# lh3/bfc

Measured on AMD Instinct MI355X. Metric: M k-mers/s counted (bloom+htab) on 150 bp reads, higher is better.
Workload: dtype u64

## Files before the change

bfc_amd/csrc/bfcg_bloom3.hip:

```cpp
#include <hip/hip_runtime.h>
#include <stdint.h>
#include <stdlib.h>
#include "kmer_dev.h"
#include "bfcg_internal.h"
#include "bfcg_dev.h"

using namespace bfcg;

#define B3_UND 0x40000000u
#define B3_SEEN16 0x8000u
#define B3_COLD_NR 8
#define B3_WALK_U 4
template <int BT, int PF, bool COLD>
__global__ __launch_bounds__(BT, PF <= 2 ? 8 : 6) void k_bloom3(KParams P, BloomArgs A)
{
	extern __shared__ __attribute__((aligned(16))) unsigned char smem[];
	__shared__ uint32_t s_list_n, s_ovf, s_pool_off, s_emit_n, s_fs_used, s_wb_n, s_pad3[2];
	const uint32_t f = blockIdx.x;
	const bool ho_log = A.ho_stride != 0;
#ifdef BFCG_MEASURE
	const long long t_start = clock64();
#endif
	const bool eager = A.eager != 0, spec = eager && A.cap2 != 0;
	constexpr int B3_SL = 1024 / BT;
	uint4 sl[B3_SL];
	uint32_t e_st = 0, e_f0 = 0, e_f2 = 0, e_c = 0, e_s = 0, e_h = 0;
	RecW<3> cur[PF], nxt[PF];
#pragma unroll
	for (int u = 0; u < PF; ++u) { cur[u].d[0] = cur[u].d[1] = cur[u].d[2] = 0; nxt[u] = cur[u]; }
#pragma unroll
	for (int j = 0; j < B3_SL; ++j) sl[j] = make_uint4(0, 0, 0, 0);
	if (eager) {
		const uint4 *src = reinterpret_cast<const uint4 *>(reinterpret_cast<const unsigned int *>(A.bloom) + (uint64_t)f * (16u << P.R));
#pragma unroll
		for (int j = 0; j < B3_SL; ++j) if ((uint32_t)(threadIdx.x + j * BT) < (4u << P.R)) sl[j] = src[threadIdx.x + j * BT];
		const uint32_t *const any = reinterpret_cast<const uint32_t *>(A.stats);
		const uint32_t *const p_st = A.sticky ? A.sticky : any, *const p_fl = A.flags ? A.flags : any;
		const uint32_t *const p_c = A.cnt2 ? A.cnt2 + f : A.start + f + 1, *const p_s = A.cap2 ? any : A.start + f, *const p_h = ho_log ? A.ho_cur + f : any;
		e_st = *p_st; e_f0 = p_fl[0]; e_f2 = p_fl[2]; e_c = *p_c; e_s = *p_s; e_h = *p_h;
		if (spec) {
			const uint32_t *r0 = A.recs + (uint64_t)(f * A.cap2) * 3;
#pragma unroll
			for (int u = 0; u < PF; ++u) { const uint32_t i = threadIdx.x + u * BT; if (i < A.cap2) cur[u] = rec_load<3>(r0 + (uint64_t)i * 3); }
		}
	}
	const bool poisoned = eager ? (((A.sticky ? e_st : 0u) | (A.flags ? e_f0 | e_f2 : 0u)) != 0u) : batch_poisoned(A);
	if (poisoned) { if (ho_log && threadIdx.x == 0) A.ho_mark[f] = A.ho_cur[f]; return; }
	uint32_t rs, n;
	if (!eager) region_list(A, f, rs, n);
	else if (A.cap2) { rs = f * A.cap2; n = e_c < A.cap2 ? e_c : A.cap2; }
	else { rs = e_s; n = A.cnt2 ? e_c : e_c - e_s; }
	if (n == 0) { if (threadIdx.x == 0) { if (ho_log) A.ho_mark[f] = A.ho_cur[f]; else if (A.agg_cnt) A.agg_cnt[f] = 0; } return; }
	uint32_t ho_cur0 = 0;
	unsigned long long *ho_base;
	if (ho_log) {
		ho_cur0 = eager ? e_h : A.ho_cur[f];
		if (ho_cur0 + n > A.ho_stride) {
			if (threadIdx.x == 0) { atomicAdd(&A.stats[(size_t)(f & (ST_SLOTS - 1)) * ST_N + ST_ERR_POOL], 1ULL); A.ho_mark[f] = ho_cur0; }
			return;
		}
		ho_base = A.ho + (uint64_t)f * A.ho_stride + ho_cur0;
	} else ho_base = reinterpret_cast<unsigned long long *>(A.stream_out) + rs;
	A.stats += (size_t)(f & (ST_SLOTS - 1)) * ST_N;
	const uint32_t region_dw = 16u << P.R;
	unsigned char *sp = smem;
	unsigned int *region = reinterpret_cast<unsigned int *>(sp); sp += (size_t)region_dw * 4;
	const uint32_t nblk = 1u << P.R;
	unsigned int *bcnt = reinterpret_cast<unsigned int *>(sp), *boff = bcnt + nblk;
	if (COLD) sp += (size_t)(2 * nblk + 4) * 4;
	unsigned int *fs = reinterpret_cast<unsigned int *>(sp); if (!COLD) sp += (size_t)P.fs_cap * 4;
	unsigned int *la = reinterpret_cast<unsigned int *>(sp); sp += (size_t)P.list_cap * 4;
	unsigned int *lb = reinterpret_cast<unsigned int *>(sp); sp += (size_t)P.list_cap * 4;
	unsigned short *lc = reinterpret_cast<unsigned short *>(sp); sp += (size_t)P.list_cap * 2;
	unsigned short *ord = reinterpret_cast<unsigned short *>(sp);
	const uint32_t fs_mask = P.fs_cap - 1;
	const uint32_t *recs = A.recs + (uint64_t)rs * 3;
	unsigned int *g_region = reinterpret_cast<unsigned int *>(A.bloom) + (uint64_t)f * region_dw;
	const uint32_t imp = (P.f_base + f) >> P.F2;
	const Dec3 D = dec3_geom(P);
	const int tid = threadIdx.x, lane = tid & 63;
	const uint32_t mask_a = (1u << D.a) - 1u, imp_sh = D.n ? imp << D.lo : 0u, sh_up = D.lo + D.n;
#ifdef BFCG_MEASURE
	const bool timing = BFCG_ABL(P, 64) && tid == 0;
	long long tq[7] = {0, 0, 0, 0, 0, 0, 0};
	long long tc[7] = {0, 0, 0, 0, 0, 0, 0};
	if (timing) tq[0] = t_start;
#define B3_TC(i) do { if (timing) tc[i] = clock64(); } while (0)
#else
#define B3_TC(i) do { } while (0)
#endif
	auto addr3 = [&](uint32_t d0, uint32_t d1) -> uint32_t {
		const uint32_t y0d = d0 & mask_a, upper = y0d >> D.up;
		const uint32_t y0lo = D.n ? (y0d & D.lowmask) | imp_sh | (upper << sh_up) : y0d;
		const uint32_t y1lo = __builtin_amdgcn_alignbit(d1, d0, D.a) & D.mk32;
		const uint32_t hh = upper | (((y0lo - y1lo) ^ y1lo) << D.sh_x);
		uint32_t h2 = (hh >> 9) & 511u;
		h2 |= (uint32_t)((h2 & 31u) == 0);
		return (y0d & D.rmask) | ((hh & 511u) << 8) | (h2 << 17);
	};
	auto entry3 = [&](uint32_t d0, uint32_t d1) -> unsigned long long {
		const unsigned long long AA = d0 | ((unsigned long long)d1 << 32);
		const unsigned long long y1 = (AA >> D.a) & ((1ULL << P.k) - 1);
		const uint32_t y0d = d0 & mask_a;
		const unsigned long long id = (unsigned long long)((y0d & D.rmask) | ((y0d >> D.up) << D.R)) | (y1 << D.sh_y1);
		return (id << 1) | (unsigned long long)((d1 >> D.sh_flag) & 1u);
	};
#pragma unroll
	for (int u = 0; u < PF; ++u) {
		const uint32_t i = tid + u * BT;
		if (!spec && i < n) cur[u] = rec_load<3>(recs + (uint64_t)i * 3);
		if (i + BT * PF < n) nxt[u] = rec_load<3>(recs + (uint64_t)(i + BT * PF) * 3);
	}
	if (spec) {
#pragma unroll
		for (int u = 0; u < PF; ++u) if ((uint32_t)(tid + u * BT) >= n) cur[u].d[0] = cur[u].d[1] = cur[u].d[2] = 0;
	}
	{
		const uint4 *src = reinterpret_cast<const uint4 *>(g_region);
		uint4 *dst = reinterpret_cast<uint4 *>(region);
		if (eager) {
#pragma unroll
			for (int j = 0; j < B3_SL; ++j) if ((uint32_t)(tid + j * BT) < region_dw / 4) dst[tid + j * BT] = sl[j];
		} else for (uint32_t i = tid; i < region_dw / 4; i += BT) dst[i] = src[i];
		if constexpr (COLD) { for (uint32_t i = tid; i < 2 * nblk + 4; i += BT) bcnt[i] = 0; }
		else {
			uint4 *f4 = reinterpret_cast<uint4 *>(fs);
			for (uint32_t i = tid; i < P.fs_cap / 4; i += BT) f4[i] = make_uint4(FS32_EMPTY, FS32_EMPTY, FS32_EMPTY, FS32_EMPTY);
		}
		if (tid == 0) { s_list_n = 0; s_emit_n = 0; s_ovf = 0; s_fs_used = 0; s_wb_n = 0; }
	}
	__syncthreads();
#ifdef BFCG_MEASURE
	if (timing) tq[1] = clock64();
#endif
	volatile uint32_t *v_ovf = &s_ovf;

	for (uint32_t base = 0; base < n; base += BT * PF) {
		uint32_t pk[PF], um[PF];
#pragma unroll
		for (int u = 0; u < PF; ++u) {
			pk[u] = 0; um[u] = 0;
			if (base + u * BT + (uint32_t)(tid & ~63) < n) {
				pk[u] = addr3(cur[u].d[0], cur[u].d[1]);
				const B3Pos b = b3_positions((pk[u] >> 8) & 511u, pk[u] >> 17);
				const uint32_t bl64 = (pk[u] & 255u) << 6;
				const uint32_t w0 = *b3_wordp(region, bl64, b.b0), w1 = *b3_wordp(region, bl64, b.b1), w2 = *b3_wordp(region, bl64, b.b2), w3 = *b3_wordp(region, bl64, b.b3);
				um[u] = (b3_bit(w0, b.b0) | (b3_bit(w1, b.b1) << 1) | (b3_bit(w2, b.b2) << 2) | (b3_bit(w3, b.b3) << 3)) ^ 15u;
			}
		}
		unsigned long long ms[PF], ml[PF];
// ... 22 lines not shown
					if constexpr (COLD) __hip_atomic_fetch_add(&bcnt[pk[u] & 255u], 1u, __ATOMIC_RELAXED, __HIP_MEMORY_SCOPE_WORKGROUP);
				}
			}
			o_s += (uint32_t)__popcll(ms[u]); o_l += (uint32_t)__popcll(ml[u]);
		}
		if (base + BT * PF < n) {
#pragma unroll
			for (int u = 0; u < PF; ++u) {
				cur[u] = nxt[u];
				const uint32_t i = base + 2 * BT * PF + tid + u * BT;
				if (i < n) nxt[u] = rec_load<3>(recs + (uint64_t)i * 3);
			}
		}
	}
	__syncthreads();
#ifdef BFCG_MEASURE
	if (timing) tq[2] = clock64();
#endif
	const uint32_t ln = s_list_n;
	const bool ovf_list = ln > P.list_cap || ln > (COLD ? (uint32_t)(B3_COLD_NR * BT) : 8191u) || n > 65535u;
	bool dirty = true;
	if constexpr (COLD) {
		if (!ovf_list) {
			B3_TC(0);
			if (tid < 64) {
				const uint32_t per = (nblk + 63u) >> 6, b0 = (uint32_t)tid * per;
				uint32_t v[4] = {0, 0, 0, 0}, sum = 0;
#pragma unroll
				for (int t = 0; t < 4; ++t) if ((uint32_t)t < per && b0 + t < nblk) { v[t] = bcnt[b0 + t]; sum += v[t]; }
				uint32_t inc = sum;
#pragma unroll
				for (int o = 1; o < 64; o <<= 1) { const uint32_t x = __shfl_up(inc, o); if (lane >= o) inc += x; }
				uint32_t run = inc - sum;
#pragma unroll
				for (int t = 0; t < 4; ++t) if ((uint32_t)t < per && b0 + t < nblk) { boff[b0 + t] = run; bcnt[b0 + t] = run; run += v[t]; }
				if (tid == 63) boff[nblk] = inc;
			}
// ... 31 lines not shown
					sx[t] = x; sw[t] = ((w >> 8) & 0x3ffffu) | (r << 18); sq[t] = lc[pos];
				}
			}
			__syncthreads();
			B3_TC(3);
#pragma unroll
			for (int t = 0; t < B3_COLD_NR; ++t) {
				if ((uint32_t)tid + (uint32_t)t * BT < ln) {
					const uint32_t r = sw[t] >> 18;
					const B3Pos b = b3_positions(sw[t] & 511u, (sw[t] >> 9) & 511u);
					la[r] = sx[t]; lb[r] = b.b0 | (b.b1 << 9) | (b.b2 << 18); ord[r] = (unsigned short)b.b3; lc[r] = (unsigned short)sq[t];
				}
			}
			__syncthreads();
			B3_TC(4);
			if ((uint32_t)tid < nblk) {
				const uint32_t bl = (uint32_t)tid, bl64 = bl << 6, s0 = boff[bl], s1 = boff[bl + 1], last = s1 - 1u;
				uint32_t pw_n[B3_WALK_U] = {0, 0, 0, 0}, p3_n[B3_WALK_U] = {0, 0, 0, 0};
				if (s0 < s1) {
#pragma unroll
					for (int u = 0; u < B3_WALK_U; ++u) { const uint32_t jj = min(s0 + (uint32_t)u, last); pw_n[u] = lb[jj]; p3_n[u] = ord[jj]; }
				}
				for (uint32_t j = s0; j < s1; j += B3_WALK_U) {
					uint32_t pw[B3_WALK_U], p3[B3_WALK_U], sn[B3_WALK_U];
#pragma unroll
					for (int u = 0; u < B3_WALK_U; ++u) { pw[u] = pw_n[u]; p3[u] = p3_n[u]; }
#pragma unroll
					for (int u = 0; u < B3_WALK_U; ++u) { const uint32_t jj = min(j + (uint32_t)(B3_WALK_U + u), last); pw_n[u] = lb[jj]; p3_n[u] = ord[jj]; }
#pragma unroll
					for (int u = 0; u < B3_WALK_U; ++u) {
// ... 139 lines not shown
						if (um & 1u) first |= fs32_lookup(fs, fs_mask, bl * 512u + b.b0) == li;
						if (um & 2u) first |= fs32_lookup(fs, fs_mask, bl * 512u + b.b1) == li;
						if (um & 4u) first |= fs32_lookup(fs, fs_mask, bl * 512u + b.b2) == li;
						if (um & 8u) first |= fs32_lookup(fs, fs_mask, bl * 512u + b.b3) == li;
						seen = !first;
					}
					if (A.seen_out) A.seen_out[la[li]] = seen ? 2 : 1;
				}
				const unsigned long long vote = __ballot(seen);
				if (vote) {
					uint32_t o = 0;
					if (lane == 0) o = atomicAdd(&s_emit_n, (uint32_t)__popcll(vote));
					o = __builtin_amdgcn_readfirstlane(o);
					if (seen) {
						const RecW<3> r = rec_load<3>(recs + (uint64_t)lc[li] * 3);
						ho_base[o + (uint32_t)__popcll(vote & ((1ULL << lane) - 1))] = entry3(r.d[0], r.d[1]);
					}
				}
			}
			for (uint32_t i = tid; i < (1u << P.R); i += BT) region[i * 16u] &= ~0xffu;
		} else if (A.seen_out) {
			for (uint32_t li = tid; li < ln; li += BT) A.seen_out[la[li]] = 1;
		}
		dirty = ln != 0;
		__syncthreads();
	} else {
		const int nh = 4;
		uint64_t want = (uint64_t)n * nh * 2;
		const uint64_t lim = (uint64_t)(1u << P.R) * 512 * 2;
		if (want > lim) want = lim;
		uint32_t cap = 1024; while (cap < want) cap <<= 1;
		if (tid == 0) {
			uint32_t sl = f & (A.pool_slices - 1);
			while (atomicCAS(&A.pool[sl], 0ULL, 1ULL) != 0ULL) sl = (sl + 1) & (A.pool_slices - 1);
			s_pool_off = sl; s_emit_n = 0;
			atomicAdd(&A.stats[ST_SLOW_BUCKETS], 1ULL);
		}
		{
			const uint4 *src = reinterpret_cast<const uint4 *>(g_region);
			uint4 *dst = reinterpret_cast<uint4 *>(region);
			for (uint32_t i = tid; i < region_dw / 4; i += BT) dst[i] = src[i];
		}
		__syncthreads();
		unsigned long long *gfs = A.pool + A.pool_slices + (uint64_t)s_pool_off * lim;
		for (uint32_t i = tid; i < cap; i += BT) gfs[i] = FS_EMPTY;
		__threadfence();
		__syncthreads();
		const uint32_t gmask = cap - 1;
		for (uint32_t i = tid; i < n; i += BT) {
			const RecW<3> r = rec_load<3>(recs + (uint64_t)i * 3);
			const uint32_t w = addr3(r.d[0], r.d[1]), bl = w & 255u;
			uint32_t z = (w >> 8) & 511u;
			for (int j = 0; j < nh; ++j) {
				const uint32_t b = bloom_next(z, w >> 17);
				if (!b3_bit(*b3_wordp(region, bl << 6, b), b)) fs_insert<true>(gfs, gmask, bl * 512 + b, r.d[2], gmask);
			}
		}
		__threadfence();
		__syncthreads();
		for (uint32_t i0 = 0; i0 < n; i0 += BT) {
// ... 7 lines not shown
				for (int j = 0; j < nh; ++j) {
					uint32_t b = bloom_next(z, w >> 17), fi;
					if (fs_lookup<true>(gfs, gmask, bl * 512 + b, fi)) {
						unresolved = true; first |= (fi == r.d[2]);
						atomicOr(b3_wordp(region, bl << 6, b), 1u << (b & 31));
					}
				}
				seen = !unresolved || !first;
				if (A.seen_out) A.seen_out[r.d[2]] = seen ? 2 : 1;
			}
			const unsigned long long vote = __ballot(seen);
			if (vote) {
				uint32_t o = 0;
				if (lane == 0) o = atomicAdd(&s_emit_n, (uint32_t)__popcll(vote));
				o = __builtin_amdgcn_readfirstlane(o);
				if (seen) ho_base[o + (uint32_t)__popcll(vote & ((1ULL << lane) - 1))] = entry3(r.d[0], r.d[1]);
			}
		}
		__syncthreads();
		if (tid == 0) { __threadfence(); atomicExch(&A.pool[s_pool_off], 0ULL); }
	}
#ifdef BFCG_MEASURE
	if (timing) tq[3] = clock64();
#endif
	if (dirty) {
		uint4 *dst = reinterpret_cast<uint4 *>(g_region);
		const uint4 *src = reinterpret_cast<const uint4 *>(region);
		for (uint32_t i = tid; i < region_dw / 4; i += BT) dst[i] = src[i];
	}
#ifdef BFCG_MEASURE
	if (timing) tq[4] = clock64();
#endif
	if (tid == 0) {
		const uint32_t ns = s_emit_n;
		if (ns) atomicAdd(&A.stats[ST_SEEN], (unsigned long long)ns);
		if (ho_log) { A.ho_cur[f] = ho_cur0 + ns; A.ho_mark[f] = ho_cur0 + ns; }
		else if (A.agg_cnt) A.agg_cnt[f] = ns;
	}
#ifdef BFCG_MEASURE
	if (timing) {
		tq[5] = clock64();
		if (BFCG_ABL(P, 128)) {
			if (COLD) for (int t = 0; t < 6; ++t) atomicAdd(&A.stats[10 + t], (unsigned long long)(tc[t + 1] - tc[t]));
		} else {
			for (int t = 0; t < 5; ++t) atomicAdd(&A.stats[10 + t], (unsigned long long)(tq[t + 1] - tq[t]));
			atomicAdd(&A.stats[15], (unsigned long long)(tq[6] - tq[2]));
		}
	}
#endif
#undef B3_TC
	(void)s_pad3;
}

namespace bfcg {

typedef void (*BloomFn)(KParams, BloomArgs);
static BloomFn bloom3_kernel(bool pf2, bool cold)
{
	if (cold) return pf2 ? k_bloom3<512, 2, true> : k_bloom3<512, 4, true>;
	return pf2 ? k_bloom3<512, 2, false> : k_bloom3<512, 4, false>;
}
static hipError_t set_bloom3_max_lds(BloomFn fn, int lds) { return hipFuncSetAttribute((const void *)fn, hipFuncAttributeMaxDynamicSharedMemorySize, lds < BLOOM3_LDS_FLOOR ? BLOOM3_LDS_FLOOR : lds); }
hipError_t set_bloom3_lds_attr(int lds)
{
	hipError_t e = hipSuccess;
	for (int i = 0; i < 4 && e == hipSuccess; ++i) e = set_bloom3_max_lds(bloom3_kernel(i & 1, i & 2), lds);
	return e;
}

void run_bloom3(const KParams &P, const BloomArgs &A, int nfine, size_t lds, hipStream_t st)
{
	static int pf = 0;
	if (!pf) { const char *e = getenv("BFCG_B3_PF"); pf = e && atoi(e) == 2 ? 2 : e && atoi(e) == 4 ? 4 : 1; }
	const bool pf2 = P.b3_cold ? P.b3_warm != 0 : pf == 2 || (pf == 1 && P.b3_warm);
	hipLaunchKernelGGL(bloom3_kernel(pf2, P.b3_cold != 0), dim3(nfine), dim3(512), lds, st, P, A);
}

}

struct Dec4 { int up, iw, is; uint32_t rmask; };
__device__ __forceinline__ Dec4 dec4_geom(const KParams &P)
{
	Dec4 g;
	g.up = P.rec_n ? P.rec_lo : P.bf_shift - 9;
	const int io = (P.k - P.rec_n) + P.k + 1;
	g.iw = io >> 5; g.is = io & 31; g.rmask = (1u << P.R) - 1u;
	return g;
}
template <int BT, int PF>
__global__ __launch_bounds__(BT, 6) void k_bloom3fm(KParams P, BloomArgs A)
// ... 200 lines not shown
```

bfc_amd/csrc/bfcg_ctx.hip:

```cpp
#include <hip/hip_runtime.h>
#include <stdint.h>
#include <stdio.h>
#include <stdlib.h>
#include <string.h>
#include <stdarg.h>
#include <sys/mman.h>
#include <time.h>
#include <vector>
#include <thread>
#include "bfc_gpu.h"
#include "bfcg_internal.h"
#include "bfc_host.h"
#include "kmer_dev.h"

using namespace bfcg;

static thread_local char g_err[512] = "";
enum { HO_MAX_PAGES = BFCG_HO_MAX_PAGES };
enum { OP_FLAG_WORDS = 12, OP_STICKY = 8 };
static double dbg_now(void) { struct timespec ts; clock_gettime(CLOCK_MONOTONIC, &ts); return ts.tv_sec + 1e-9 * ts.tv_nsec; }
static inline void set_seg_shift(KParams &P, int s, int blk_max) { P.seg_shift = s; P.seg_blk = s < blk_max ? s : blk_max; }
int bfcg::fail(const char *fmt, ...)
{
	va_list ap; va_start(ap, fmt); vsnprintf(g_err, sizeof(g_err), fmt, ap); va_end(ap);
// ... 43 lines not shown
	int seg_total_max;
	int seg_blk_max;
	int b3_ok;
	uint32_t fs_cap_w, list_cap_w;
	uint32_t list_cap_cw;
	uint32_t list_cap_c;
	int seg_init_shift;
	int seg_escaped;
	uint64_t n_seg_grow;
	int onepass_ok, onepass;
	uint32_t *op_cursor[2], *op_seg[2], *op_flags, *h_flags[2];
	int unfinished, unfinished_mg;
	uint32_t *h_rows[2]; int rows_slot;
	uint32_t op_cap; uint64_t op_min_pos;
	int eager;
	uint32_t *cnt2; uint32_t cap2; uint64_t recs2_n;
	struct opq_t { const uint8_t *seq, *qual; uint64_t n_pos; int slot; const void *recv; int mg; uint64_t call; } opq[4]; int n_opq;
	int mg_op2_ok, mg_op2, mg_op2_allowed; uint32_t *mg_seg[4];
	int mg_slab_ok; int mg_seg_slab[4];
	uint64_t n_replayed;
	int reused;
	int seg_no_grow;
	int seg_cap_shift;
	unsigned long long *ho, *ho_keys, *h_ho_keys[2]; uint32_t *ho_cur, *ho_mark; uint32_t ho_stride; int ho_K;
	int ho_pending;
	uint64_t ho_page_call[HO_MAX_PAGES];
	int slot_commit[2]; uint64_t slot_page_call[2][HO_MAX_PAGES];
	int slot_all_committed[2];
	uint64_t keys_known;
	int commit_absorbed;
// ... 147 lines not shown
		}
		{
			const size_t room = (size_t)P.fs_cap * 4 + (size_t)P.list_cap * 8;
			uint32_t ct = 1; while ((size_t)ct * 2 * 8 <= room) ct <<= 1;
			P.ct_cap = ct;
		}
	}
	P.tab_cshift = prm->tab_cshift > 0 ? prm->tab_cshift : (P.l_pre <= 20 ? 5 : 3);
	if (prm->tab_cshift <= 0)
		while ((1ULL << (P.l_pre + P.tab_cshift)) < prm->max_batch_pos / 4 && P.l_pre + P.tab_cshift < 34) ++P.tab_cshift;
	P.track = (prm->track_order && !prm->filter_mode) ? 1 : 0;
	{ const char *e = getenv("BFCG_BT"); P.bloom_bt = e ? atoi(e) : (bloom_lds_bytes(P) > 80 * 1024 && !P.track && P.n_hashes == 4) ? 1024 : 512; if (P.bloom_bt != 1024 || P.track || P.n_hashes != 4) P.bloom_bt = 512; }
	c->n_ranks = n_ranks; c->rank = prm->rank; c->log2n = log2n;
	{ const char *e = getenv("BFCG_PIPELINE"); c->pipeline = e ? atoi(e) != 0 : prm->max_batch_pos <= (1ULL << 28); }
	{ const char *e = getenv("BFCG_EAGER"); c->eager = e ? atoi(e) != 0 : -1; }

	if (n_ranks > 1 && log2n > P.F1) { fail("multi-GPU needs a two-level partition with 2^F1=%d >= n_ranks (bf_shift=%d is too small)", 1 << P.F1, P.bf_shift); bfcg_destroy(c); return NULL; }
	P.idx_rank = n_ranks > 1 ? (uint32_t)prm->rank << (32 - log2n) : 0u;
	c->bloom_bytes = (1ULL << (P.bf_shift - 3)) >> log2n;

	BatchBufs &B = c->B;
	B.max_kmers = prm->max_batch_pos;
	const int nb1 = 1 << P.F1, nfine = (1 << P.F) >> log2n;
	c->recv_cap = n_ranks > 1 ? B.max_kmers + B.max_kmers / 4 + (1u << 20) : B.max_kmers;
	BFCG_CKN(bfcg_destroy(c), hipStreamCreate(&c->st)); BFCG_CKN(bfcg_destroy(c), hipStreamCreate(&c->stA)); BFCG_CKN(bfcg_destroy(c), hipStreamCreate(&c->stC));
	for (int b = 0; b < 2; ++b) {
		for (int i = 0; i < 7; ++i) BFCG_CKN(bfcg_destroy(c), hipEventCreate(&c->evt[b][i]));
		BFCG_CKN(bfcg_destroy(c), hipEventCreateWithFlags(&c->evA[b], hipEventDisableTiming)); BFCG_CKN(bfcg_destroy(c), hipEventCreateWithFlags(&c->evB[b], hipEventDisableTiming));
	}
	BFCG_CKN(bfcg_destroy(c), hipEventCreateWithFlags(&c->evCopy, hipEventDisableTiming));
// ... 585 lines not shown

static int opq_push(bfcg_ctx_t *c, int b, const StageB &w)
{
	if (c->n_opq == 4) return fail("internal: one-pass queue overflow");
	int mg = 0;
	if (w.recv) {
		const size_t words = (size_t)c->n_ranks * (size_t)((1 << c->P.F1) >> c->log2n) * (w.sizes_slab ? 8 : 1);
		for (;; ++mg) { int used = 0; for (int i = 0; i < c->n_opq; ++i) used |= c->opq[i].mg == mg + 1; if (!used) break; }
		if (w.sizes) memcpy(c->mg_seg[mg], w.sizes, sizeof(uint32_t) * words); else memset(c->mg_seg[mg], 0, sizeof(uint32_t) * words);
		c->mg_seg_slab[mg++] = w.sizes_slab;
	}
	c->opq[c->n_opq++] = bfcg_ctx::opq_t{w.seq, w.qual, w.pos, b, w.recv, mg, w.call};
	return 0;
}

static int enqueue_stage_b(bfcg_ctx_t *c, int b, BatchBufs &Bt, const KParams &Pt, const StageB &w)
{
	if (handover_begin(c, Bt, b, w.slabs, w.call) != 0) return -1;
	Bt.eager = c->eager >= 0 ? c->eager : w.pos >= (uint64_t)16 * nfine(c);
	run_stage_b(Pt, Bt, w.in1, w.seg_beg, w.seg_end, w.n_seg, w.segs_per_bucket, w.row_base, w.bucket_start, w.rec_bound, c->st, c->evt[b]);
	if (handover_end(c, Bt, b) != 0) return -1;
	if (w.queued) {
		BFCG_CK(hipMemcpyAsync(c->h_flags[b] + 1, c->op_flags + OP_STICKY, sizeof(uint32_t), hipMemcpyDeviceToHost, c->st));
		if (opq_push(c, b, w) != 0) return -1;
	}
	BFCG_CK(hipMemcpyAsync(c->h_snap[b], c->B.stats, sizeof(unsigned long long) * ST_N * (ST_SLOTS + 1), hipMemcpyDeviceToHost, c->st));
	c->slot_call[b] = c->call_no = w.call; c->slot_pos[b] = w.pos;
	BFCG_CK(hipEventRecord(c->evB[b], c->st));
	BFCG_CK(hipGetLastError());
	c->used[b] = 1;
	++c->n_batches;
	return w.finalise ? finalise_previous(c, b) : 0;
}

// ... 714 lines not shown
```

bfc_amd/csrc/bfcg_dev.h:

```cpp
#pragma once
#include <hip/hip_runtime.h>
#include <stdint.h>
#include "kmer_dev.h"
#include "bfcg_internal.h"

using namespace bfcg;

template <int RD> struct RecW { uint32_t d[RD]; };

template <int RD> __device__ __forceinline__ RecW<RD> rec_load(const uint32_t *p);
template <> __device__ __forceinline__ RecW<3> rec_load<3>(const uint32_t *p)
{ const uint3 v = *reinterpret_cast<const uint3 *>(p); RecW<3> r; r.d[0] = v.x; r.d[1] = v.y; r.d[2] = v.z; return r; }
template <> __device__ __forceinline__ RecW<4> rec_load<4>(const uint32_t *p)
{ const uint4 v = *reinterpret_cast<const uint4 *>(p); RecW<4> r; r.d[0] = v.x; r.d[1] = v.y; r.d[2] = v.z; r.d[3] = v.w; return r; }
template <> __device__ __forceinline__ RecW<5> rec_load<5>(const uint32_t *p)
{ RecW<5> r; r.d[0] = p[0]; r.d[1] = p[1]; r.d[2] = p[2]; r.d[3] = p[3]; r.d[4] = p[4]; return r; }
template <int RD> __device__ __forceinline__ void rec_store(uint32_t *p, const RecW<RD> &r);
template <> __device__ __forceinline__ void rec_store<3>(uint32_t *p, const RecW<3> &r)
{ *reinterpret_cast<uint3 *>(p) = make_uint3(r.d[0], r.d[1], r.d[2]); }
template <> __device__ __forceinline__ void rec_store<4>(uint32_t *p, const RecW<4> &r)
{ *reinterpret_cast<uint4 *>(p) = make_uint4(r.d[0], r.d[1], r.d[2], r.d[3]); }
template <> __device__ __forceinline__ void rec_store<5>(uint32_t *p, const RecW<5> &r)
{ p[0] = r.d[0]; p[1] = r.d[1]; p[2] = r.d[2]; p[3] = r.d[3]; p[4] = r.d[4]; }

// ... 48 lines not shown
	uint8_t *seen_out;
	uint64_t *agg_out;
	uint32_t *agg_cnt;
	uint32_t *stream_out;
	unsigned long long *seg_tab;
	uint32_t n_fine;
	TabOrder ord;
	unsigned long long batch_hi;
	const uint32_t *cnt2; uint32_t cap2;
	unsigned long long *ho; uint32_t ho_stride; uint32_t *ho_cur; uint32_t *ho_mark;
	uint32_t ho_pages, ho_mark_stride;
	unsigned long long *ho_keys;
	const uint32_t *flags;
	const uint32_t *sticky;
	uint32_t eager;
};

__device__ __forceinline__ void region_list(const BloomArgs &A, uint32_t f, uint32_t &rs, uint32_t &n)
{
	if (A.cap2) { const uint32_t c = A.cnt2[f]; rs = f * A.cap2; n = c < A.cap2 ? c : A.cap2; }
	else if (A.cnt2) { rs = A.start[f]; n = A.cnt2[f]; }
	else { rs = A.start[f]; n = A.start[f + 1] - rs; }
}
__device__ __forceinline__ bool batch_poisoned(const BloomArgs &A) { return (A.sticky && *A.sticky) || (A.flags && (A.flags[0] | A.flags[2])); }


struct Dec3 { int ok, a, lo, n, up, sh_x, R, sh_flag, sh_y1; uint32_t lowmask, rmask, mk32; };
__device__ __forceinline__ Dec3 dec3_geom(const KParams &P)
{
	Dec3 g;
// ... 89 lines not shown
```

bfc_amd/csrc/bfcg_internal.h:

```cpp
#pragma once
#include <hip/hip_runtime.h>
#define BFCG_TILE1 4096
#define BFCG_BT1 256
#define BFCG_SCAN_CH 64
static inline int bfcg_rec_dwords(int k, int rec_n) { const int bits = 2 * k - rec_n + 33; return bits <= 96 ? 3 : bits <= 128 ? 4 : 5; }
static constexpr int bfcg_tile_of_rw(int rw) { return rw == 5 ? 2048 : rw == 4 ? 3072 : 4096; }
static constexpr int bfcg_tile1_of_rw(int rw) { return rw == 3 ? 4096 : 3072; }
#define BFCG_MAXB 1024
#define BFCG_HO_MAX_PAGES 8
#ifdef BFCG_MEASURE
#define BFCG_ABL(P, bits) ((P).ablate & (bits))
#else
#define BFCG_ABL(P, bits) 0
#endif
#include <stdint.h>
struct bfcg_ctx; struct bfcg_kcov;

extern "C" void bfcg_set_error(const char *msg);
extern "C" void *bfcg_bloom_slice(struct bfcg_ctx *c, int which, uint64_t *bytes);
extern "C" int bfcg_resident_register(const void *bf, void *dev, int device, int n_shift);

#define BFCG_UT_NBUF 24
struct bfcg_kmers {
	int k, l_pre, cshift, device, owns_table;
// ... 57 lines not shown
	uint32_t *start1, *row_base;
	uint32_t *rows2, *start2;
	uint64_t *recs1, *recs2;
	uint64_t max_kmers;
	unsigned long long *bloom, *bloom_hi, *table;
	unsigned long long *stats;
	uint64_t *tab_ovf; uint32_t tab_ovf_cap;
	unsigned long long *pool; uint32_t pool_slices;
	uint8_t *seen_out;
	uint64_t *agg_out; uint32_t *agg_cnt;
	uint32_t *stream_out; int stream;
	uint32_t *op_cursor, *op_flags, *op_sticky, *op_seg; uint32_t op_cap;
	uint32_t op_own_lo, op_own_n, op_own_delta;
	uint32_t *cnt2; uint32_t cap2;
	int eager;
	uint32_t *cnt_live;
	unsigned long long *ho; uint32_t ho_stride; uint32_t *ho_cur, *ho_mark; uint32_t ho_mark_stride, ho_page; int ho_commit; unsigned long long *ho_keys;
	unsigned long long *seg_tab;
	unsigned long long *tab_first, *sub_last;
	unsigned long long batch_hi;
};

void run_stage_a(const KParams &P, const BatchBufs &B, const uint8_t *seq, const uint8_t *qual, int64_t n_pos, uint64_t *out1, hipStream_t st, hipEvent_t *ev);
void run_stage_a_onepass(const KParams &P, const BatchBufs &B, const uint8_t *seq, const uint8_t *qual, int64_t n_pos, uint64_t *out1, hipStream_t st, hipEvent_t *ev);
void run_stage_b(const KParams &P, const BatchBufs &B, const uint64_t *in1, const uint32_t *seg_beg, const uint32_t *seg_end, int n_seg, int segs_per_bucket,
                 const uint32_t *row_base, const uint32_t *bucket_start, uint64_t n_rec_bound, hipStream_t st, hipEvent_t *ev);
void run_pack_rows(const KParams &P, const BatchBufs &B, int n_ranks, uint32_t row_w, uint32_t *rows, hipStream_t st);
void run_seg_setup_mg(const KParams &P, int rw_dwords, const uint32_t *rows, uint32_t row_w, int n_ranks, int s_lo, int s_hi, uint32_t cap, uint32_t *seg, unsigned long long *total, hipStream_t st);
void run_batch(const KParams &P, const BatchBufs &B, const uint8_t *seq, const uint8_t *qual, int64_t n_pos, hipStream_t st, hipEvent_t *ev);
int bloom_lds_bytes(const KParams &P);
// ... 64 lines not shown
```

bfc_amd/csrc/bfcg_kernels.hip:

```cpp
#include <hip/hip_runtime.h>
#include <stdint.h>
#include <stdlib.h>
#include <string.h>
#include <stdio.h>
#include "kmer_dev.h"
#include "bfcg_internal.h"
#include "bfcg_dev.h"
#include "bfcg_k1.h"

using namespace bfcg;

#define WAVE 64








template <typename W> __device__ __forceinline__ uint32_t fine_id(const KParams &P, uint64_t y0, uint64_t y1)
{
	W m = kmask<W>(P.k);
	uint64_t hash = bloom_hash<W>(P.k, (W)y0, (W)y1, m);
// ... 1977 lines not shown
	return {(const uint32_t *)B.recs2, B.start2};
}

template <typename W, int RW>
static BloomArgs run_bloom_t(const KParams &P, const BatchBufs &B, const uint32_t *fine_recs, const uint32_t *fine_start, int nfine, hipStream_t st)
{
	BloomArgs A;
	memset(&A, 0, sizeof(A));
	A.recs = fine_recs; A.start = fine_start; A.bloom = B.bloom; A.bloom_hi = B.bloom_hi; A.table = B.table; A.stats = B.stats;
	A.tab_ovf = B.tab_ovf; A.tab_ovf_cap = B.tab_ovf_cap; A.ovf_cnt = B.stats + (size_t)ST_SLOTS * ST_N; A.pool = B.pool; A.pool_slices = B.pool_slices; A.seen_out = B.seen_out;
	A.agg_out = B.agg_out; A.agg_cnt = B.agg_cnt; A.n_fine = (uint32_t)nfine; A.stream_out = nullptr; A.seg_tab = nullptr;
	A.ord.first = B.tab_first; A.ord.sub_last = B.sub_last; A.batch_hi = B.batch_hi;
	A.cnt2 = nullptr; A.cap2 = 0; A.flags = B.op_flags; A.sticky = B.op_sticky;
	if (P.F2 > 0 && B.cap2) { A.cnt2 = B.cnt2; A.cap2 = B.cap2; }
	else if (P.F2 > 0 && B.cnt_live) A.cnt2 = B.cnt_live;
	A.eager = B.eager != 0;
	const bool h4 = P.n_hashes == 4;
	if (P.filter_mode && B.bloom_hi) {
		if (RW == 4 && P.b3fm) run_bloom3fm(P, A, nfine, (size_t)bloom_lds_bytes(P), st);
		else launch_bloom<W, RW>(!h4 ? BV_FM_ANYH : P.bloom_bt == 1024 ? BV_FM_1024 : BV_FM, P, A, nfine, st);
	} else if (P.seg && B.seg_tab && (B.stream_out || B.ho)) {
		A.stream_out = B.stream_out; A.seg_tab = B.seg_tab; A.table = nullptr; A.agg_out = nullptr;
		A.ho = B.ho; A.ho_stride = B.ho_stride; A.ho_cur = B.ho_cur; A.ho_mark = B.ho_stride ? B.ho_mark + (size_t)B.ho_page * B.ho_mark_stride : nullptr;
		if (RW == 3 && P.b3 && (P.b3_cold || !P.dedupe)) run_bloom3(P, A, nfine, (size_t)bloom_lds_bytes(P), st);
		else launch_bloom<W, RW>(!h4 ? BV_SEG_ANYH : RW == 3 && bloom_fast3(P) ? BV_SEG_F3 : BV_SEG, P, A, nfine, st);
	} else if (B.stream && B.stream_out && !P.track && h4) {
		A.stream_out = B.stream_out;
		launch_bloom<W, RW>(BV_STREAM, P, A, nfine, st);
	} else if (P.track) launch_bloom<W, RW>(h4 ? BV_TRACK : BV_TRACK_ANYH, P, A, nfine, st);
	else launch_bloom<W, RW>(!h4 ? BV_ANYH : P.bloom_bt == 1024 ? BV_1024 : BV_512, P, A, nfine, st);
	return A;
// ... 157 lines not shown
```

Baseline: 42960.

## Let bloom3 blocks process a span of regions with next-region prefetch

New measurement: 40570. -5.6%, worse.

```diff
diff --git a/bfc_amd/csrc/bfcg_bloom3.hip b/bfc_amd/csrc/bfcg_bloom3.hip
--- a/bfc_amd/csrc/bfcg_bloom3.hip
+++ b/bfc_amd/csrc/bfcg_bloom3.hip
@@ -16,56 +16,14 @@
 {
 	extern __shared__ __attribute__((aligned(16))) unsigned char smem[];
 	__shared__ uint32_t s_list_n, s_ovf, s_pool_off, s_emit_n, s_fs_used, s_wb_n, s_pad3[2];
-	const uint32_t f = blockIdx.x;
 	const bool ho_log = A.ho_stride != 0;
-#ifdef BFCG_MEASURE
-	const long long t_start = clock64();
-#endif
 	const bool eager = A.eager != 0, spec = eager && A.cap2 != 0;
 	constexpr int B3_SL = 1024 / BT;
-	uint4 sl[B3_SL];
-	uint32_t e_st = 0, e_f0 = 0, e_f2 = 0, e_c = 0, e_s = 0, e_h = 0;
-	RecW<3> cur[PF], nxt[PF];
-#pragma unroll
-	for (int u = 0; u < PF; ++u) { cur[u].d[0] = cur[u].d[1] = cur[u].d[2] = 0; nxt[u] = cur[u]; }
-#pragma unroll
-	for (int j = 0; j < B3_SL; ++j) sl[j] = make_uint4(0, 0, 0, 0);
-	if (eager) {
-		const uint4 *src = reinterpret_cast<const uint4 *>(reinterpret_cast<const unsigned int *>(A.bloom) + (uint64_t)f * (16u << P.R));
-#pragma unroll
-		for (int j = 0; j < B3_SL; ++j) if ((uint32_t)(threadIdx.x + j * BT) < (4u << P.R)) sl[j] = src[threadIdx.x + j * BT];
-		const uint32_t *const any = reinterpret_cast<const uint32_t *>(A.stats);
-		const uint32_t *const p_st = A.sticky ? A.sticky : any, *const p_fl = A.flags ? A.flags : any;
-		const uint32_t *const p_c = A.cnt2 ? A.cnt2 + f : A.start + f + 1, *const p_s = A.cap2 ? any : A.start + f, *const p_h = ho_log ? A.ho_cur + f : any;
-		e_st = *p_st; e_f0 = p_fl[0]; e_f2 = p_fl[2]; e_c = *p_c; e_s = *p_s; e_h = *p_h;
-		if (spec) {
-			const uint32_t *r0 = A.recs + (uint64_t)(f * A.cap2) * 3;
-#pragma unroll
-			for (int u = 0; u < PF; ++u) { const uint32_t i = threadIdx.x + u * BT; if (i < A.cap2) cur[u] = rec_load<3>(r0 + (uint64_t)i * 3); }
-		}
-	}
-	const bool poisoned = eager ? (((A.sticky ? e_st : 0u) | (A.flags ? e_f0 | e_f2 : 0u)) != 0u) : batch_poisoned(A);
-	if (poisoned) { if (ho_log && threadIdx.x == 0) A.ho_mark[f] = A.ho_cur[f]; return; }
-	uint32_t rs, n;
-	if (!eager) region_list(A, f, rs, n);
-	else if (A.cap2) { rs = f * A.cap2; n = e_c < A.cap2 ? e_c : A.cap2; }
-	else { rs = e_s; n = A.cnt2 ? e_c : e_c - e_s; }
-	if (n == 0) { if (threadIdx.x == 0) { if (ho_log) A.ho_mark[f] = A.ho_cur[f]; else if (A.agg_cnt) A.agg_cnt[f] = 0; } return; }
-	uint32_t ho_cur0 = 0;
-	unsigned long long *ho_base;
-	if (ho_log) {
-		ho_cur0 = eager ? e_h : A.ho_cur[f];
-		if (ho_cur0 + n > A.ho_stride) {
-			if (threadIdx.x == 0) { atomicAdd(&A.stats[(size_t)(f & (ST_SLOTS - 1)) * ST_N + ST_ERR_POOL], 1ULL); A.ho_mark[f] = ho_cur0; }
-			return;
-		}
-		ho_base = A.ho + (uint64_t)f * A.ho_stride + ho_cur0;
-	} else ho_base = reinterpret_cast<unsigned long long *>(A.stream_out) + rs;
-	A.stats += (size_t)(f & (ST_SLOTS - 1)) * ST_N;
-	const uint32_t region_dw = 16u << P.R;
+	constexpr bool B3_PRE_SL = !(COLD && PF <= 2), B3_PRE_RECS = !COLD && PF <= 2;
+	const uint32_t span = A.span > 1u ? A.span : 1u, f_first = blockIdx.x * span;
+	const uint32_t region_dw = 16u << P.R, nblk = 1u << P.R;
 	unsigned char *sp = smem;
 	unsigned int *region = reinterpret_cast<unsigned int *>(sp); sp += (size_t)region_dw * 4;
-	const uint32_t nblk = 1u << P.R;
 	unsigned int *bcnt = reinterpret_cast<unsigned int *>(sp), *boff = bcnt + nblk;
 	if (COLD) sp += (size_t)(2 * nblk + 4) * 4;
 	unsigned int *fs = reinterpret_cast<unsigned int *>(sp); if (!COLD) sp += (size_t)P.fs_cap * 4;
@@ -74,19 +32,91 @@
 	unsigned short *lc = reinterpret_cast<unsigned short *>(sp); sp += (size_t)P.list_cap * 2;
 	unsigned short *ord = reinterpret_cast<unsigned short *>(sp);
 	const uint32_t fs_mask = P.fs_cap - 1;
+	const Dec3 D = dec3_geom(P);
+	const uint32_t mask_a = (1u << D.a) - 1u, sh_up = D.lo + D.n;
+	const uint32_t *const any = reinterpret_cast<const uint32_t *>(A.stats);
+	volatile uint32_t *v_ovf = &s_ovf;
+	uint4 sl[B3_SL];
+#pragma unroll
+	for (int j = 0; j < B3_SL; ++j) sl[j] = make_uint4(0, 0, 0, 0);
+	uint32_t e_c = 0, e_s = 0, e_h = 0;
+	RecW<3> cur[PF], nxt[PF];
+	auto request = [&](uint32_t ff, bool recs_too, uint32_t t) __attribute__((always_inline)) {
+		const uint32_t *const p_c = A.cnt2 ? A.cnt2 + ff : A.start + ff + 1, *const p_s = A.cap2 ? any : A.start + ff, *const p_h = ho_log ? A.ho_cur + ff : any;
+		e_c = *p_c; e_s = *p_s; e_h = *p_h;
+		const uint4 *src = reinterpret_cast<const uint4 *>(reinterpret_cast<const unsigned int *>(A.bloom) + (uint64_t)ff * (16u << P.R));
+#pragma unroll
+		for (int j = 0; j < B3_SL; ++j) { sl[j] = make_uint4(0, 0, 0, 0); if ((uint32_t)(t + j * BT) < (4u << P.R)) sl[j] = src[t + j * BT]; }
+		if (recs_too) {
+			const uint32_t *r0 = A.recs + (uint64_t)(ff * A.cap2) * 3;
+#pragma unroll
+			for (int u = 0; u < PF; ++u) { const uint32_t i = t + u * BT; if (i < A.cap2) cur[u] = rec_load<3>(r0 + (uint64_t)i * 3); }
+		}
+	};
+
+	bool poisoned = false;
+	bool pre = false;
+	bool have_cur = false;
+	for (uint32_t g = 0; g < span; ++g) {
+	const uint32_t f = f_first + g;
+	int tid = threadIdx.x;
+	asm volatile("" : "+v"(tid));
+	const int lane = tid & 63;
+	if (f >= A.n_fine) break;
+#ifdef BFCG_MEASURE
+	const long long t_start = clock64();
+#endif
+	const bool first_of_span = !pre;
+	if (!B3_PRE_RECS || !pre) {
+#pragma unroll
+		for (int u = 0; u < PF; ++u) cur[u].d[0] = cur[u].d[1] = cur[u].d[2] = 0;
+	}
+	if (!pre) {
+#pragma unroll
+		for (int j = 0; j < B3_SL; ++j) sl[j] = make_uint4(0, 0, 0, 0);
+		e_c = e_s = e_h = 0; have_cur = false;
+		if (!poisoned) {
+			have_cur = spec;
+			if (eager) {
+				const uint32_t *const p_st = A.sticky ? A.sticky : any, *const p_fl = A.flags ? A.flags : any;
+				const uint32_t e_st = *p_st, e_f0 = p_fl[0], e_f2 = p_fl[2];
+				request(f, spec, (uint32_t)tid);
+				poisoned = __builtin_amdgcn_readfirstlane((A.sticky ? e_st : 0u) | (A.flags ? e_f0 | e_f2 : 0u)) != 0u;
+			} else poisoned = batch_poisoned(A);
+		}
+	}
+	pre = false;
+	e_c = __builtin_amdgcn_readfirstlane(e_c); e_s = __builtin_amdgcn_readfirstlane(e_s); e_h = __builtin_amdgcn_readfirstlane(e_h);
+	if (poisoned) { if (ho_log && threadIdx.x == 0) A.ho_mark[f] = A.ho_cur[f]; continue; }
+	uint32_t rs, n;
+	if (!eager) region_list(A, f, rs, n);
+	else if (A.cap2) { rs = f * A.cap2; n = e_c < A.cap2 ? e_c : A.cap2; }
+	else { rs = e_s; n = A.cnt2 ? e_c : e_c - e_s; }
+	rs = __builtin_amdgcn_readfirstlane(rs); n = __builtin_amdgcn_readfirstlane(n);
+	if (n == 0) { if (threadIdx.x == 0) { if (ho_log) A.ho_mark[f] = A.ho_cur[f]; else if (A.agg_cnt) A.agg_cnt[f] = 0; } continue; }
+	uint32_t ho_cur0 = 0;
+	unsigned long long *ho_base;
+	if (ho_log) {
+		ho_cur0 = __builtin_amdgcn_readfirstlane(eager ? e_h : A.ho_cur[f]);
+		if (ho_cur0 + n > A.ho_stride) {
+			if (threadIdx.x == 0) { atomicAdd(&A.stats[(size_t)(f & (ST_SLOTS - 1)) * ST_N + ST_ERR_POOL], 1ULL); A.ho_mark[f] = ho_cur0; }
+			continue;
+		}
+		ho_base = A.ho + (uint64_t)f * A.ho_stride + ho_cur0;
+	} else ho_base = reinterpret_cast<unsigned long long *>(A.stream_out) + rs;
+	unsigned long long *const st_row = A.stats + (size_t)(f & (ST_SLOTS - 1)) * ST_N;
 	const uint32_t *recs = A.recs + (uint64_t)rs * 3;
 	unsigned int *g_region = reinterpret_cast<unsigned int *>(A.bloom) + (uint64_t)f * region_dw;
 	const uint32_t imp = (P.f_base + f) >> P.F2;
-	const Dec3 D = dec3_geom(P);
-	const int tid = threadIdx.x, lane = tid & 63;
-	const uint32_t mask_a = (1u << D.a) - 1u, imp_sh = D.n ? imp << D.lo : 0u, sh_up = D.lo + D.n;
+	const uint32_t imp_sh = D.n ? imp << D.lo : 0u;
 #ifdef BFCG_MEASURE
-	const bool timing = BFCG_ABL(P, 64) && tid == 0;
+	const bool timing = BFCG_ABL(P, 64) && tid == 0 && !(BFCG_ABL(P, 256) && first_of_span);
 	long long tq[7] = {0, 0, 0, 0, 0, 0, 0};
 	long long tc[7] = {0, 0, 0, 0, 0, 0, 0};
 	if (timing) tq[0] = t_start;
 #define B3_TC(i) do { if (timing) tc[i] = clock64(); } while (0)
 #else
+	(void)first_of_span;
 #define B3_TC(i) do { } while (0)
 #endif
 	auto addr3 = [&](uint32_t d0, uint32_t d1) -> uint32_t {
@@ -108,13 +138,15 @@
 #pragma unroll
 	for (int u = 0; u < PF; ++u) {
 		const uint32_t i = tid + u * BT;
-		if (!spec && i < n) cur[u] = rec_load<3>(recs + (uint64_t)i * 3);
+		if (!have_cur && i < n) cur[u] = rec_load<3>(recs + (uint64_t)i * 3);
+		nxt[u].d[0] = nxt[u].d[1] = nxt[u].d[2] = 0;
 		if (i + BT * PF < n) nxt[u] = rec_load<3>(recs + (uint64_t)(i + BT * PF) * 3);
 	}
-	if (spec) {
+	if (have_cur) {
 #pragma unroll
 		for (int u = 0; u < PF; ++u) if ((uint32_t)(tid + u * BT) >= n) cur[u].d[0] = cur[u].d[1] = cur[u].d[2] = 0;
 	}
+	if (g) __syncthreads();
 	{
 		const uint4 *src = reinterpret_cast<const uint4 *>(g_region);
 		uint4 *dst = reinterpret_cast<uint4 *>(region);
@@ -125,7 +157,9 @@
 		if constexpr (COLD) { for (uint32_t i = tid; i < 2 * nblk + 4; i += BT) bcnt[i] = 0; }
 		else {
 			uint4 *f4 = reinterpret_cast<uint4 *>(fs);
-			for (uint32_t i = tid; i < P.fs_cap / 4; i += BT) f4[i] = make_uint4(FS32_EMPTY, FS32_EMPTY, FS32_EMPTY, FS32_EMPTY);
+			uint32_t fe = FS32_EMPTY;
+			asm volatile("" : "+v"(fe));
+			for (uint32_t i = tid; i < P.fs_cap / 4; i += BT) f4[i] = make_uint4(fe, fe, fe, fe);
 		}
 		if (tid == 0) { s_list_n = 0; s_emit_n = 0; s_ovf = 0; s_fs_used = 0; s_wb_n = 0; }
 	}
@@ -133,7 +167,6 @@
 #ifdef BFCG_MEASURE
 	if (timing) tq[1] = clock64();
 #endif
-	volatile uint32_t *v_ovf = &s_ovf;
 
 	for (uint32_t base = 0; base < n; base += BT * PF) {
 		uint32_t pk[PF], um[PF];
@@ -186,6 +219,20 @@
 		}
 	}
 	__syncthreads();
+#define B3_AHEAD() do { \
+		if constexpr (B3_PRE_SL) { \
+			if constexpr (B3_PRE_RECS) { _Pragma("unroll") for (int u = 0; u < PF; ++u) cur[u].d[0] = cur[u].d[1] = cur[u].d[2] = 0; } \
+			if (eager && g + 1 < span && f + 1 < A.n_fine) { \
+				have_cur = B3_PRE_RECS && spec; \
+				request(f + 1, have_cur, (uint32_t)tid); \
+				pre = true; \
+			} else {  \
+				_Pragma("unroll") for (int j = 0; j < B3_SL; ++j) sl[j] = make_uint4(0, 0, 0, 0); \
+				e_c = e_s = e_h = 0; have_cur = false; \
+			} \
+		} \
+	} while (0)
+	if constexpr (!COLD) B3_AHEAD();
 #ifdef BFCG_MEASURE
 	if (timing) tq[2] = clock64();
 #endif
@@ -193,6 +240,7 @@
 	const bool ovf_list = ln > P.list_cap || ln > (COLD ? (uint32_t)(B3_COLD_NR * BT) : 8191u) || n > 65535u;
 	bool dirty = true;
 	if constexpr (COLD) {
+		if (ovf_list) B3_AHEAD();
 		if (!ovf_list) {
 			B3_TC(0);
 			if (tid < 64) {
@@ -254,6 +302,7 @@
 			}
 			__syncthreads();
 			B3_TC(4);
+			B3_AHEAD();
 			if ((uint32_t)tid < nblk) {
 				const uint32_t bl = (uint32_t)tid, bl64 = bl << 6, s0 = boff[bl], s1 = boff[bl + 1], last = s1 - 1u;
 				uint32_t pw_n[B3_WALK_U] = {0, 0, 0, 0}, p3_n[B3_WALK_U] = {0, 0, 0, 0};
@@ -423,7 +472,7 @@
 					o = __builtin_amdgcn_readfirstlane(o);
 					if (seen) {
 						const RecW<3> r = rec_load<3>(recs + (uint64_t)lc[li] * 3);
-						ho_base[o + (uint32_t)__popcll(vote & ((1ULL << lane) - 1))] = entry3(r.d[0], r.d[1]);
+						ho_base[o + (uint32_t)__builtin_amdgcn_mbcnt_hi((uint32_t)(vote >> 32), __builtin_amdgcn_mbcnt_lo((uint32_t)vote, 0u))] = entry3(r.d[0], r.d[1]);
 					}
 				}
 			}
@@ -440,10 +489,10 @@
 		if (want > lim) want = lim;
 		uint32_t cap = 1024; while (cap < want) cap <<= 1;
 		if (tid == 0) {
-			uint32_t sl = f & (A.pool_slices - 1);
-			while (atomicCAS(&A.pool[sl], 0ULL, 1ULL) != 0ULL) sl = (sl + 1) & (A.pool_slices - 1);
-			s_pool_off = sl; s_emit_n = 0;
-			atomicAdd(&A.stats[ST_SLOW_BUCKETS], 1ULL);
+			uint32_t ps = f & (A.pool_slices - 1);
+			while (atomicCAS(&A.pool[ps], 0ULL, 1ULL) != 0ULL) ps = (ps + 1) & (A.pool_slices - 1);
+			s_pool_off = ps; s_emit_n = 0;
+			atomicAdd(&st_row[ST_SLOW_BUCKETS], 1ULL);
 		}
 		{
 			const uint4 *src = reinterpret_cast<const uint4 *>(g_region);
@@ -452,7 +501,9 @@
 		}
 		__syncthreads();
 		unsigned long long *gfs = A.pool + A.pool_slices + (uint64_t)s_pool_off * lim;
-		for (uint32_t i = tid; i < cap; i += BT) gfs[i] = FS_EMPTY;
+		uint32_t ge = 0xffffffffu;
+		asm volatile("" : "+v"(ge));
+		for (uint32_t i = tid; i < cap; i += BT) gfs[i] = ((unsigned long long)ge << 32) | ge;
 		__threadfence();
 		__syncthreads();
 		const uint32_t gmask = cap - 1;
@@ -490,7 +541,7 @@
 				uint32_t o = 0;
 				if (lane == 0) o = atomicAdd(&s_emit_n, (uint32_t)__popcll(vote));
 				o = __builtin_amdgcn_readfirstlane(o);
-				if (seen) ho_base[o + (uint32_t)__popcll(vote & ((1ULL << lane) - 1))] = entry3(r.d[0], r.d[1]);
+				if (seen) ho_base[o + (uint32_t)__builtin_amdgcn_mbcnt_hi((uint32_t)(vote >> 32), __builtin_amdgcn_mbcnt_lo((uint32_t)vote, 0u))] = entry3(r.d[0], r.d[1]);
 			}
 		}
 		__syncthreads();
@@ -509,7 +560,7 @@
 #endif
 	if (tid == 0) {
 		const uint32_t ns = s_emit_n;
-		if (ns) atomicAdd(&A.stats[ST_SEEN], (unsigned long long)ns);
+		if (ns) atomicAdd(&st_row[ST_SEEN], (unsigned long long)ns);
 		if (ho_log) { A.ho_cur[f] = ho_cur0 + ns; A.ho_mark[f] = ho_cur0 + ns; }
 		else if (A.agg_cnt) A.agg_cnt[f] = ns;
 	}
@@ -517,14 +568,16 @@
 	if (timing) {
 		tq[5] = clock64();
 		if (BFCG_ABL(P, 128)) {
-			if (COLD) for (int t = 0; t < 6; ++t) atomicAdd(&A.stats[10 + t], (unsigned long long)(tc[t + 1] - tc[t]));
+			if (COLD) for (int t = 0; t < 6; ++t) atomicAdd(&st_row[10 + t], (unsigned long long)(tc[t + 1] - tc[t]));
 		} else {
-			for (int t = 0; t < 5; ++t) atomicAdd(&A.stats[10 + t], (unsigned long long)(tq[t + 1] - tq[t]));
-			atomicAdd(&A.stats[15], (unsigned long long)(tq[6] - tq[2]));
+			for (int t = 0; t < 5; ++t) atomicAdd(&st_row[10 + t], (unsigned long long)(tq[t + 1] - tq[t]));
+			atomicAdd(&st_row[15], (unsigned long long)(tq[6] - tq[2]));
 		}
 	}
 #endif
 #undef B3_TC
+#undef B3_AHEAD
+	}
 	(void)s_pad3;
 }
 
@@ -549,7 +602,10 @@
 	static int pf = 0;
 	if (!pf) { const char *e = getenv("BFCG_B3_PF"); pf = e && atoi(e) == 2 ? 2 : e && atoi(e) == 4 ? 4 : 1; }
 	const bool pf2 = P.b3_cold ? P.b3_warm != 0 : pf == 2 || (pf == 1 && P.b3_warm);
-	hipLaunchKernelGGL(bloom3_kernel(pf2, P.b3_cold != 0), dim3(nfine), dim3(512), lds, st, P, A);
+	BloomArgs As = A;
+	As.span = A.eager && A.span > 1 ? A.span : 1u;
+	while (As.span > 1 && ((uint32_t)nfine % As.span || (As.span & (As.span - 1)))) As.span >>= 1;
+	hipLaunchKernelGGL(bloom3_kernel(pf2, P.b3_cold != 0), dim3((uint32_t)nfine / As.span), dim3(512), lds, st, P, As);
 }
 
 }
diff --git a/bfc_amd/csrc/bfcg_ctx.hip b/bfc_amd/csrc/bfcg_ctx.hip
--- a/bfc_amd/csrc/bfcg_ctx.hip
+++ b/bfc_amd/csrc/bfcg_ctx.hip
@@ -81,6 +81,7 @@
 	uint32_t *h_rows[2]; int rows_slot;
 	uint32_t op_cap; uint64_t op_min_pos;
 	int eager;
+	int b3_span;
 	uint32_t *cnt2; uint32_t cap2; uint64_t recs2_n;
 	struct opq_t { const uint8_t *seq, *qual; uint64_t n_pos; int slot; const void *recv; int mg; uint64_t call; } opq[4]; int n_opq;
 	int mg_op2_ok, mg_op2, mg_op2_allowed; uint32_t *mg_seg[4];
@@ -258,6 +259,7 @@
 	c->n_ranks = n_ranks; c->rank = prm->rank; c->log2n = log2n;
 	{ const char *e = getenv("BFCG_PIPELINE"); c->pipeline = e ? atoi(e) != 0 : prm->max_batch_pos <= (1ULL << 28); }
 	{ const char *e = getenv("BFCG_EAGER"); c->eager = e ? atoi(e) != 0 : -1; }
+	{ const char *e = getenv("BFCG_B3_SPAN"); const int s = e ? atoi(e) : 0; c->b3_span = s == 1 || s == 2 || s == 4 || s == 8 ? s : 0; }
 
 	if (n_ranks > 1 && log2n > P.F1) { fail("multi-GPU needs a two-level partition with 2^F1=%d >= n_ranks (bf_shift=%d is too small)", 1 << P.F1, P.bf_shift); bfcg_destroy(c); return NULL; }
 	P.idx_rank = n_ranks > 1 ? (uint32_t)prm->rank << (32 - log2n) : 0u;
@@ -873,10 +875,13 @@
 	return 0;
 }
 
+#define B3_SPAN_COLD 1
+#define B3_SPAN_WARM 1
 static int enqueue_stage_b(bfcg_ctx_t *c, int b, BatchBufs &Bt, const KParams &Pt, const StageB &w)
 {
 	if (handover_begin(c, Bt, b, w.slabs, w.call) != 0) return -1;
 	Bt.eager = c->eager >= 0 ? c->eager : w.pos >= (uint64_t)16 * nfine(c);
+	Bt.b3_span = !Bt.eager ? 1 : c->b3_span ? c->b3_span : Pt.b3_cold ? B3_SPAN_COLD : B3_SPAN_WARM;
 	run_stage_b(Pt, Bt, w.in1, w.seg_beg, w.seg_end, w.n_seg, w.segs_per_bucket, w.row_base, w.bucket_start, w.rec_bound, c->st, c->evt[b]);
 	if (handover_end(c, Bt, b) != 0) return -1;
 	if (w.queued) {
diff --git a/bfc_amd/csrc/bfcg_dev.h b/bfc_amd/csrc/bfcg_dev.h
--- a/bfc_amd/csrc/bfcg_dev.h
+++ b/bfc_amd/csrc/bfcg_dev.h
@@ -86,6 +86,7 @@
 	const uint32_t *flags;
 	const uint32_t *sticky;
 	uint32_t eager;
+	uint32_t span;
 };
 
 __device__ __forceinline__ void region_list(const BloomArgs &A, uint32_t f, uint32_t &rs, uint32_t &n)
diff --git a/bfc_amd/csrc/bfcg_internal.h b/bfc_amd/csrc/bfcg_internal.h
--- a/bfc_amd/csrc/bfcg_internal.h
+++ b/bfc_amd/csrc/bfcg_internal.h
@@ -95,6 +95,7 @@
 	uint32_t op_own_lo, op_own_n, op_own_delta;
 	uint32_t *cnt2; uint32_t cap2;
 	int eager;
+	int b3_span;
 	uint32_t *cnt_live;
 	unsigned long long *ho; uint32_t ho_stride; uint32_t *ho_cur, *ho_mark; uint32_t ho_mark_stride, ho_page; int ho_commit; unsigned long long *ho_keys;
 	unsigned long long *seg_tab;
diff --git a/bfc_amd/csrc/bfcg_kernels.hip b/bfc_amd/csrc/bfcg_kernels.hip
--- a/bfc_amd/csrc/bfcg_kernels.hip
+++ b/bfc_amd/csrc/bfcg_kernels.hip
@@ -2015,7 +2015,7 @@
 	A.cnt2 = nullptr; A.cap2 = 0; A.flags = B.op_flags; A.sticky = B.op_sticky;
 	if (P.F2 > 0 && B.cap2) { A.cnt2 = B.cnt2; A.cap2 = B.cap2; }
 	else if (P.F2 > 0 && B.cnt_live) A.cnt2 = B.cnt_live;
-	A.eager = B.eager != 0;
+	A.eager = B.eager != 0; A.span = B.eager && B.b3_span > 1 ? (uint32_t)B.b3_span : 1u;
 	const bool h4 = P.n_hashes == 4;
 	if (P.filter_mode && B.bloom_hi) {
 		if (RW == 4 && P.b3fm) run_bloom3fm(P, A, nfine, (size_t)bloom_lds_bytes(P), st);
```
